# AlexanderGSC/gmres

Measured on AMD Instinct MI355X. Metric: Arnoldi iters/sec + HBM GB/s, 4096² Poisson-2D fp64, GMRES(m=95), higher is better.
Workload: dtype f64

## Files before the change

### gmres_amd/__init__.py

```python
from ._native import GkError, peer_info, runtime_info
from .solver import (MGSR_MF, MGSR_OMP, PREC, Context, LocalGroup, SolveResult, gmres_hh, gmres_mgsr, pbicgstab,
                     SrSolve, cb_plan_query, pcg, res_plan_query, slab_partition)

__all__ = ["GkError", "Context", "LocalGroup", "SolveResult", "gmres_mgsr", "gmres_hh", "slab_partition", "pcg", "pbicgstab", "MGSR_OMP", "MGSR_MF", "PREC",
           "res_plan_query", "cb_plan_query", "runtime_info", "SrSolve", "peer_info"]
```

### gmres_amd/_native.py

```python
from __future__ import annotations

import ctypes
import os
import sys
import re

PKG = os.path.dirname(os.path.abspath(__file__))
LIB_DIR = os.environ.get("GK_LIB_DIR") or os.path.join(PKG, "lib")
HIP_SO = os.path.join(LIB_DIR, "libgmres_hip.so")
FHOST_SO = os.path.join(LIB_DIR, "libgmres_fhost.so")
HEADER = os.path.join(os.path.dirname(PKG), "include", "gmres_hip.h")

GK_OK = 0
GK_ERR_COMM = -6
GK_TUNE_PROJ_NT = 0
GK_TUNE_STENCIL_BLOCKS = 2
GK_TUNE_SR_BLOCKS = 28
GK_TUNE_SR_TWO_LEVEL = 29
GK_TUNE_XCHG_TIMEOUT_MS = 7
GK_TUNE_RES, GK_TUNE_RES_R2, GK_TUNE_RES_SHARE, GK_TUNE_RES_TIMEOUT_MS = 8, 9, 10, 11
GK_TUNE_VERR_ORDER = 14
GK_TUNE_HH_FUSE = 15
GK_TUNE_CHEB_STEN = 16
GK_TUNE_SPIN_WAIT = 18
GK_TUNE_GRAPH = 19
GK_TUNE_RES_QDEF = 20
GK_TUNE_RES_PC = 21
GK_TUNE_RES_FOLD = 22
GK_TUNE_RES_BLOCK = 23
GK_TUNE_WATCHDOG_MS = 24
GK_TUNE_HH_NORM_ORDER = 25
GK_TUNE_RES_PF = 27
GK_TUNE_RES_PIPE = 30
GK_TUNE_RIGHT_FUSED = 31
GK_TUNE_RES_PIPE_CARRY = 32
GK_SIDE_LEFT, GK_SIDE_RIGHT = 0, 1
GK_BASIS_F64, GK_BASIS_F32 = 0, 1
GK_ERR_ARG, GK_ERR_STATE = -1, -4
GK_PREC_IDENTITY, GK_PREC_CBPR2, GK_PREC_CHEB = 0, 1, 2
(GK_KID_PROJ, GK_KID_STENCIL, GK_KID_SCALE, GK_KID_UPDATE, GK_KID_COMM, GK_KID_OTHER, GK_KID_RES, GK_KID_PREC,
 GK_KID_HALO, GK_KID_GRAPH) = range(10)
GK_KID_SR = 10
SR_PASS_NAMES = ["sr_cg_p", "sr_cg_x", "sr_cg_z", "sr_bi_p", "sr_bi_pc", "sr_bi_s", "sr_bi_sc", "sr_st1", "sr_st2",
                 "sr_bi_x", "sr_bi_pe", "sr_bi_se", "sr_dot", "sr_cg_xz", "sr_bi_pz", "sr_bi_sz"]
KID_NAMES = ["proj", "stencil", "scale", "update", "comm", "other", "res", "prec", "halo", "graph"] + SR_PASS_NAMES
GK_SR_PCG, GK_SR_BICGSTAB = 0, 1
COMM_KINDS = {0: None, 1: "rccl", 2: "local-group", 3: "xgmi-device-exchange"}
GK_RES_CB = 7
RES_VARIANTS = {0: None, 1: "prefetch", 2: "pairs", 3: "pairs+lds", 4: "w-only", 5: "w+column", 6: "blocked",
                GK_RES_CB: "compressed-basis"}
# ... 64 lines not shown
    "gk_hh_step_async": (c_int, [c_vp, c_int, c_int]),
    "gk_hh_step_wait": (c_int, [c_vp, c_int, _dp]),
    "gk_hh_update_x": (c_int, [c_vp, _dp, c_int]),
    "gk_hh_verr": (c_int, [c_vp, c_int, _dp]),
    "gk_profile_enable": (c_int, [c_vp, c_int]),
    "gk_profile_reset": (c_int, [c_vp]),
    "gk_profile_read": (c_int, [c_vp, c_int, _dp, ctypes.POINTER(c_ll)]),
    "gk_sync": (c_int, [c_vp]),
    "gk_debug_hold_stream": (c_int, [c_vp, c_int]),
    "gk_profile_res_wg": (c_int, [c_vp, c_int, _dp, _dp, c_int, _ip]),
    "gk_profile_res_trace": (c_int, [c_vp, c_int, c_int, c_int, c_vp, c_int, c_int, _ip, _ip, _dp]),
    "gk_profile_res_split": (c_int, [c_vp, c_int, c_int, _dp, _dp, _dp, ctypes.POINTER(c_ll)]),
    "gk_set_tuning": (c_int, [c_vp, c_int, c_int]),
    "gk_res_plan_query": (c_int, [c_ll, c_int, c_int, c_int, c_int, c_int, ctypes.POINTER(c_ll)]),
    "gk_res_info": (c_int, [c_vp, c_int, ctypes.POINTER(c_ll)]),
    "gk_lanczos_bounds": (c_int, [c_vp, c_int, _dp, _dp]),
    "gk_vec_count": (c_int, [c_vp, _ip]),
    "gk_vec_apply": (c_int, [c_vp, c_int, c_int, c_int]),
    "gk_vec_dot": (c_int, [c_vp, c_int, c_int, _dp]),
    "gk_vec_lincomb": (c_int, [c_vp, c_int, c_int, c_int, c_int, c_int, c_double, c_double]),
    "gk_sr_start": (c_int, [c_vp, c_int, c_double, c_int]),
    "gk_sr_iterate": (c_int, [c_vp, c_int]),
    "gk_sr_status": (c_int, [c_vp, c_int, _ip, _ip, _dp]),
    "gk_sr_history": (c_int, [c_vp, _dp, c_int]),
    "gk_poisson5": (c_int, [c_int, c_int, c_vp, c_vp, c_vp, c_vp, c_vp]),
    "gk_precond_apply": (c_int, [c_int, c_int, _dp, c_int, c_vp, c_vp, c_vp, c_vp]),
    "gk_mgs_project": (c_int, [c_ll, c_vp, c_vp, c_vp, c_vp]),
    "gk_dot": (c_int, [c_ll, c_vp, c_vp, c_vp, c_vp]),
}

# ... 123 lines not shown
```

### gmres_amd/csrc/gk_api.hip

```cpp
#include <dlfcn.h>

#include <algorithm>
#include <cmath>
#include <cstdarg>
#include <cstdio>
#include <cstdlib>
#include <cstring>

#include "gk_blk.hpp"
#include "gk_cb.hpp"
#include "gk_host.hpp"
#include "gk_kernels.hpp"
#include "gk_resident.hpp"

using namespace gkh;
using gk::nt_auto_for;
using gk::plan_info;
using gk::plan_resident;
using gk::ResPlan;
using gk::RES_R2_BIG;

namespace gkh __attribute__((visibility("hidden"))) {

thread_local std::string g_err;
// ... 233 lines not shown
bool res_plan(gk_ctx *c, ResPlan &p, bool hh = false) {
    if (c->tune_res == 0 || c->res_broken || c->m > gk::RHMAX || c->res_cus <= 0 || c->res_gath == nullptr)
        return false;
    if (collective(c) && !(c->xs_on && c->nranks > 1)) return false;
    if (c->tune_res < 0 && c->res_share > 1) return false;
    const int gmax = std::max(1, std::min(gk::RGMAX, c->res_cus / std::max(1, c->res_share)));
    const int cap = c->tune_res_r2 > 0 ? c->tune_res_r2 : RES_R2_BIG;
    plan_resident(c->nloc, gmax, cap, c->tune_res_wonly, hh,
                  c->tune_nt > 0 || (c->tune_nt < 0 && c->nt_auto), p, c->tune_res_pc, c->tune_res_blk, c->tune_res_pf,
                  c->tune_res_pipe, c->tune_res_carry);
    if (c->nranks > 1) p.carry = 0;
    if (p.wo && !hh && c->m + 1 > gk::WO_HMAX) return false;
    return true;
}

enum { RESF_CLOSE_HH = 1, RESF_UNIT_INIT = 2, RESF_PIN_LOCAL = 4 };
int res_step(gk_ctx *c, int j, const ResPlan &p, const double *pin, int npin, double *hs, double *hcopy,
             int mode = gk::RES_MGS, double *w = nullptr, i64 unit_g = -1, int flags = 0) {
    ProfScope ps(c, GK_KID_RES);
    const bool close = (flags & RESF_CLOSE_HH) && mode == gk::RES_HH_UP;
    if ((flags & ~RESF_PIN_LOCAL) != 0 && !p.wo)
        return set_err(GK_ERR_STATE, "resident flags %d need the w-only variant", flags);
    const bool pin_local = (flags & RESF_PIN_LOCAL) && mode != gk::RES_HH_DOWN && c->xs_on && c->nranks > 1;
    const int np = (mode == gk::RES_MGS ? (p.bvar >= 0 ? gk::blk_exchanges(j, p.blk) : 2 * j) : j) + (close ? 1 : 0);
    if (c->res_tag > 0xF0000000u) {
        HIPCHK(hipMemsetAsync(c->res_gath, 0, sizeof(gk::u64) * gk::RES_GATH_ALL, c->st));
        c->res_tag = 1;
    }
    gk::ResArgs a{};
    a.w = w != nullptr ? w : c->w;
    a.mode = mode;
    a.coef = mode == gk::RES_MGS ? 1.0 : 2.0;
    a.tail0 = mode == gk::RES_HH_UP ? (i64)j - c->g0 : 0;
    a.V = c->V;
    a.vout = c->V + (i64)j * c->ld;
    a.ld = c->ld;
    a.pin = pin;
    a.npin = npin;
    a.hs = hs;
    a.hcopy = hcopy;
    a.gath = c->res_gath;
    a.gm = c->res_gm;
    a.j = j;
    a.n = c->nloc;
    a.nres2 = p.nres2;
    a.r2e = p.r2e;
    a.l2e = p.l2e;
    a.unit_known = mode == gk::RES_HH_DOWN && unit_g >= 0;
    a.unit_e = (a.unit_known && unit_g >= c->g0 && unit_g < c->g0 + c->nloc) ? unit_g - c->g0 : -1;
    a.unit_init = a.unit_known && (flags & RESF_UNIT_INIT) ? 1 : 0;
    a.close_hh = close ? 1 : 0;
    a.hb = c->hb;
    a.tag0 = c->res_tag;
    c->res_tag += (unsigned)np;
    a.timeout = (gk::u64)c->res_timeout_ms * (gk::u64)c->xs_tick_per_ms;
    a.err = c->res_err_dev;
    a.stamps = c->res_split ? c->res_stamps : nullptr;
    if (c->res_trace != nullptr && j == c->res_trace_j && mode == c->res_trace_mode) {
        a.trace = c->res_trace;
        c->res_trace_g = p.G;
        c->res_trace_np = np;
    }
    a.qdef = c->tune_res_qdef != 0 ? 1 : 0;
    a.nranks = 1;
    if (c->xs_on && c->nranks > 1) {
        a.err = c->xs_err_dev;
        a.timeout = std::max(a.timeout, c->xs_timeout);
// ... 843 lines not shown
    CHK(check_ctx(c));
    if (j < 1 || j > c->m) return set_err(GK_ERR_ARG, "step j=%d outside 1..%d", j, c->m);
    if (!c->cycle_mgs) return set_err(GK_ERR_STATE, "gk_mgs_step before gk_mgs_cycle_start");
    HIPCHK(hipSetDevice(c->dev));
    const i64 ld = c->ld;
    double *V = c->V;
    const int m2 = c->m + 2;
    double *hs = c->hall + (i64)(j - 1) * m2;
    c->prof_on_step = (j % c->prof_every) == 0;
    const int s0 = 0;
    ResPlan rp;
    gk::CbPlan cp;
    const bool cb = cb_on(c);
    const bool res = cb ? cb_plan_ctx(c, cp) : res_plan(c, rp);
    const double *vj = cb ? cb_vjw(c) : V + (i64)(j - 1) * ld, *v1 = cb ? cb_v1w(c) : V;
    if (right_prec(c))
        CHK(op_right(c, vj, c->w, gk::ACC_DOT, v1, slot(c, s0)));
    else
        CHK(op_precond(c, vj, c->w, false, gk::ACC_DOT, v1, slot(c, s0)));
    int np = c->last_np;
    if (res && cb) {
        CHK(cb_step(c, j, cp, slot(c, s0), np, hs, c->hallh_dev + (i64)(j - 1) * m2));
        HIPCHK(hipEventRecord(c->ev_step[j], c->st));
        c->prof_on_step = true;
        return GK_OK;
    }
    if (res) {
        const bool fold = c->tune_res_fold && c->xs_on && c->nranks > 1;
        if (!fold) CHK(allreduce(c, slot(c, s0), np));
        CHK(res_step(c, j, rp, slot(c, s0), np, hs, c->hallh_dev + (i64)(j - 1) * m2, gk::RES_MGS, nullptr, -1,
// ... 376 lines not shown
            xs_set_timeout(c, value);
            break;
        case GK_TUNE_RES: c->tune_res = value < 0 ? -1 : (value != 0); break;
        case GK_TUNE_RES_R2:
            if (value != 0 && value != 2 && value != 4 && value != 8 && value != 12)
                return set_err(GK_ERR_ARG, "resident cap must be 0 (auto), 2, 4, 8 or 12");
            c->tune_res_r2 = value;
            break;
        case GK_TUNE_RES_SHARE:
            if (value < 1) return set_err(GK_ERR_ARG, "share must be >= 1");
            c->res_share = value;
            break;
        case GK_TUNE_RES_WONLY: c->tune_res_wonly = value < 0 ? -1 : (value != 0); break;
        case GK_TUNE_RES_PIPE: c->tune_res_pipe = value < 0 ? -1 : (value != 0); break;
        case GK_TUNE_RES_PIPE_CARRY: c->tune_res_carry = value < 0 ? -1 : (value != 0); break;
        case GK_TUNE_HH_FUSE: c->tune_hh_fuse = value != 0; break;
        case GK_TUNE_CHEB_STEN: c->tune_cheb_sten = value != 0; break;
        case GK_TUNE_SPIN_WAIT: c->tune_spin_wait = value != 0; break;
        case GK_TUNE_GRAPH: c->tune_graph = value != 0; break;
        case GK_TUNE_RES_QDEF: c->tune_res_qdef = value < 0 ? -1 : (value != 0); break;
        case GK_TUNE_RES_PC: c->tune_res_pc = value < 0 ? -1 : (value != 0); break;
        case GK_TUNE_RES_FOLD: c->tune_res_fold = value != 0; break;
        case GK_TUNE_WATCHDOG_MS: c->watchdog_ms = std::max(0, value); break;
        case GK_TUNE_HH_NORM_ORDER: c->tune_hh_norm_order = value != 0; break;
        case GK_TUNE_RES_BLOCK:
            if (value != 1 && value != 2 && value != 4)
                return set_err(GK_ERR_ARG, "GK_TUNE_RES_BLOCK %d: blocks of 1 (strict MGS-R), 2 or 4 projections", value);
            if (c->cycle_mgs)
                c->pend_res_blk = value;
            else
// ... 209 lines not shown
            info[gk::RPI_L2E] = cp.l2e;
            info[gk::RPI_LDS] = cp.lds;
            info[gk::RPI_NRES2] = cp.nres2;
            info[gk::RPI_WT] = gk::CB_WT;
            info[gk::RPI_BLK] = 1;
        }
    }
    int cs = c->pkind == GK_PREC_CHEB && c->tune_cheb_sten && c->pdeg <= gk::CF_LMAX && c->N >= gk::CF_PTS &&
             c->tune_cheb_fused && c->N % 2 == 0 &&
             (i64)c->N * std::max(c->nlines, c->max_lines) * 8 < (1LL << 31);
    if (cs && collective(c) && c->nranks > 1) cs = c->min_lines == 0 ? -1 : (c->min_lines >= c->pdeg + 1 ? 1 : 0);
    info[gk::RPI_CHEB_STEN] = cs;
    return GK_OK;
}

}


namespace gkh __attribute__((visibility("hidden"))) {
double *g_scratch[64] = {nullptr};

int stateless_ctx(gk_ctx &c, int N, int nlines, i64 n, void *stream) {
    int dev = 0;
    HIPCHK(hipGetDevice(&dev));
    if (dev < 0 || dev >= 64) return set_err(GK_ERR_ARG, "device id %d", dev);
    if (g_scratch[dev] == nullptr) {
        if (hipMalloc(&g_scratch[dev], sizeof(double) * (NSLOT * gk::NPMAX + 64)) != hipSuccess)
            return set_err(GK_ERR_NOMEM, "scratch allocation failed");
    }
    c.dev = dev;
// ... 248 lines not shown
```

### gmres_amd/csrc/gk_host.hpp

```cpp
#pragma once
#include <hip/hip_runtime.h>
#include <rccl/rccl.h>

#include <condition_variable>
#include <deque>
#include <mutex>
#include <string>
#include <vector>

#include "../../include/gmres_hip.h"
#include "gk_res.hpp"

using gk::i64;

namespace gk {
struct SrDev;
struct SrMirror;
}

struct gk_group {
    int n = 0;
    std::mutex mu;
    std::condition_variable cv;
    int arrived = 0;
// ... 51 lines not shown
    gk::u64 *res_gath = nullptr;
    double *res_gm = nullptr;
    int tune_res_blk = 1;
    int tune_res_pf = 0;
    int pend_res_blk = 0, pend_res_pf = -1;
    int watchdog_ms = 0;
    bool broken = false;
    unsigned *hold_word = nullptr, *hold_word_dev = nullptr;
    int *res_err = nullptr, *res_err_dev = nullptr;
    unsigned res_tag = 1;
    int res_cus = 0;
    int tune_res = -1;
    int tune_res_r2 = 0;
    int tune_res_pipe = -1;
    int tune_res_carry = -1;
    int tune_res_wonly = -1;
    int tune_verr_order = 1;
    int tune_hh_fuse = 1;
    int tune_hh_norm_order = 0;
    int res_share = 1;
    int res_timeout_ms = 20000;
    bool res_broken = false;
    gk::u64 *res_stamps = nullptr;
    bool res_split = false;
    gk::u64 *res_trace = nullptr;
    int res_trace_j = 0, res_trace_mode = -1;
    int res_trace_g = 0, res_trace_np = 0;
    int vec = 2, JT = 16;
    dim3 sgrid;
    int sr_JT = 64, tune_sr_blocks = 0;
// ... 117 lines not shown
```

### gmres_amd/csrc/gk_res.hpp

```cpp
#pragma once
#include "gk_common.hpp"
#include "gk_cheb.hpp"

namespace gk {

constexpr int XS_MAXR = 16;
constexpr int XS_MAXV = 128;
constexpr i64 XS_RED_WORDS = 2LL * XS_MAXR * XS_MAXV * 2;
typedef unsigned long long u64;
struct XsPeers {
    u64 *p[XS_MAXR];
};
enum { XS_SLAB = 0, XS_VEC = 1, XS_BCAST = 2 };

__device__ __forceinline__ void xs_put(u64 *q, unsigned seq, unsigned data) {
    __hip_atomic_store(q, ((u64)seq << 32) | data, __ATOMIC_RELAXED, __HIP_MEMORY_SCOPE_SYSTEM);
}

__device__ __forceinline__ int xs_flag(const int *err) {
    return __hip_atomic_load(err, __ATOMIC_RELAXED, __HIP_MEMORY_SCOPE_SYSTEM);
}

enum { XG_ABORT = -1, XG_LATE = 0, XG_OK = 1 };
__device__ __forceinline__ int xs_get(const u64 *q, unsigned seq, u64 deadline, unsigned *data, const int *err) {
// ... 39 lines not shown
    int unit_known;
    int r2e, l2e;
    XsPeers peers;
    int nranks, rank;
    unsigned xseq0;
    int mode;
    double coef;
    i64 tail0;
    u64 *stamps;
    int close_hh;
    double *hb;
    int unit_init;
    u64 *trace;
    int qdef;
    int pin_local;
    double *gm;
};
constexpr int RES_TRACE_X = 2 * RHMAX + 2;

struct ResClock {
    u64 t0 = 0, tp = 0, pass = 0, wait = 0;
    __device__ __forceinline__ void start(const u64 *st) {
        if (st != nullptr) t0 = tp = wall_clock64();
    }
    __device__ __forceinline__ void passed(const u64 *st) {
        if (st != nullptr) {
            const u64 n = wall_clock64();
            pass += n - tp;
            tp = n;
        }
    }
    __device__ __forceinline__ void waited(const u64 *st) {
        if (st != nullptr) {
            const u64 n = wall_clock64();
            wait += n - tp;
            tp = n;
        }
    }
    __device__ __forceinline__ void finish(u64 *st, int mode) {
        if (st != nullptr && threadIdx.x == 0) {
            u64 *q = st + 4 * ((i64)mode * RGMAX + blockIdx.x);
            q[0] += pass;
            q[1] += wait;
            q[2] += wall_clock64() - t0;
            q[3] += 1;
        }
    }
};

enum { RES_MGS = 0, RES_HH_UP = 1, RES_HH_DOWN = 2 };
enum { RK_NONE = 0, RK_DOT = 1, RK_NORM = 2 };

__device__ __forceinline__ unsigned res_stream_wg() { return gridDim.x - 1 - blockIdx.x; }
// ... 274 lines not shown
```

### gmres_amd/csrc/gk_resident.hip

```cpp
#include <hip/hip_runtime.h>

#include <algorithm>
#include <atomic>
#include <cstdarg>
#include <cstdio>

#include "../../include/gmres_hip.h"
#include "gk_blk.hpp"
#include "gk_res.hpp"
#include "gk_resident.hpp"

namespace gk {

template <int R2, int L2, bool PF, bool NT, bool CW, int MODE>
__global__ __launch_bounds__(RT, 2) void k_mgs_res(ResArgs a) {
    extern __shared__ double2 lw[];
    __shared__ double sm[RWAVES];
    __shared__ double bc[1];
    __shared__ int okf;
    __shared__ double hsh[RHMAX + 1];
    constexpr int RB = PF ? R2 : 1;
    constexpr int DT = CW ? RT - 64 : RT;
    const int t = threadIdx.x;
    const bool data = !CW || t >= 64;
// ... 291 lines not shown
static_assert(PIPE_CARRY >= 0 && PIPE_CARRY <= PIPE_D, "GK_RES_PIPE_CARRY: 0 .. GK_RES_PIPE_D chunks of the ring");
#ifndef GK_RES_TOUCH_MGS_CARRY
#define GK_RES_TOUCH_MGS_CARRY 20
#endif
constexpr int TOUCH_MGS_CARRY = GK_RES_TOUCH_MGS_CARRY;

template <class F, int... I>
__device__ __forceinline__ void seq_apply(F &&f, std::integer_sequence<int, I...>) {
    (f(std::integral_constant<int, I>{}), ...);
}
template <int N, class F>
__device__ __forceinline__ void seq_for(F &&f) {
    seq_apply(f, std::make_integer_sequence<int, N>{});
}

template <int RW, int LW, int MODE, int WBT = WB, bool PIPE = false, int CARRY = 0>
__global__ __launch_bounds__(WT, 1) void k_mgs_wres(ResArgs a) {
    static_assert(CARRY >= 0 && CARRY <= WBT && (CARRY == 0 || (PIPE && MODE == RES_MGS && CARRY <= RW)),
                  "carried chunks: a head of the pipelined pass's ring, register chunks of the MGS step");
    extern __shared__ double2 lw[];
    __shared__ double sm[WT / 64];
    __shared__ double bc[1];
    __shared__ int okf;
    __shared__ int xdone;
    __shared__ double hsh[MODE == RES_MGS ? WO_HMAX : 1];
    const int t = threadIdx.x;
    constexpr int mode = MODE;
    constexpr int PACE = MODE == RES_MGS ? TOUCH_PACE : TOUCH_PACE_HH;
    constexpr int TCH = MODE == RES_MGS ? (PIPE ? (CARRY > 0 ? TOUCH_MGS_CARRY : TOUCH_MGS_PIPE) : TOUCH_MGS) : TOUCH;
    const int j = a.j, np = res_np(mode, j);
    const i64 n2 = a.n >> 1, ld2 = a.ld >> 1;
    const i64 nch = a.nres2 / WT;
// ... 7 lines not shown
    clk.start(a.stamps);
    int touch_sink = 0;
    const i64 sstride = (i64)gridDim.x * WT;
    const i64 sbase = a.nres2 + (i64)res_stream_wg() * WT + t;
    double2 wr[RW];
    [[maybe_unused]] d2v ra[CARRY > 0 ? WBT : 1], rb[CARRY > 0 ? WBT : 1];
    if (mode == RES_HH_DOWN && a.unit_init) {
        const i64 u = a.unit_e;
        auto unit2 = [&](i64 e2) { return double2{2 * e2 == u ? 1.0 : 0.0, 2 * e2 + 1 == u ? 1.0 : 0.0}; };
#pragma unroll
        for (int k = 0; k < RW; ++k) wr[k] = (c0 + k < cend) ? unit2((c0 + k) * WT + t) : double2{0.0, 0.0};
        for (int k = 0; k < LW; ++k)
            if (l0 + k < lend) lw[k * WT + t] = unit2((l0 + k) * WT + t);
        for (i64 e = sbase; e < n2; e += sstride) W2[e] = unit2(e);
        if ((a.n & 1) && blockIdx.x == gridDim.x - 1 && t == 0) a.w[a.n - 1] = (a.n - 1 == u) ? 1.0 : 0.0;
    } else {
#pragma unroll
        for (int k = 0; k < RW; ++k) wr[k] = (PIPE || c0 + k < cend) ? W2[(c0 + k) * WT + t] : double2{0.0, 0.0};
        for (int k = 0; k < LW; ++k)
            if (PIPE || l0 + k < lend) lw[k * WT + t] = W2[(l0 + k) * WT + t];
    }
    auto red = [&](double &acc, const double2 &v, const double2 &b, int kind, i64 e2, bool chk) {
        if (kind == RK_DOT) {
            acc = acc + v.x * b.x;
            acc = acc + v.y * b.y;
        } else if (kind == RK_NORM) {
            sq_acc(acc, v, e2, tail0, chk);
        }
    };
    const i64 wc0 = c0, wl0 = l0;
// ... 130 lines not shown
                    wv[u].y = wv[u].y - ch * av[u].y;
                    W2[e] = wv[u];
                    red(acc, wv[u], bv[u], kind, e, mode == RES_HH_UP && 2 * a.nres2 < tail0);
                }
            }
        }
        if ((a.n & 1) && blockIdx.x == gridDim.x - 1 && t == 0) {
            const i64 e = a.n - 1;
            const double x = a.w[e] - ch * a.V[(i64)i * a.ld + e];
            a.w[e] = x;
            if (kind == RK_DOT) acc = acc + x * a.V[(i64)q * a.ld + e];
            if (kind == RK_NORM && e >= tail0) acc = acc + x * x;
        }
        return acc;
    };
    [[maybe_unused]] auto head = [&](int pn) {
        int zero = 0;
        asm volatile("" : "+s"(zero));
        const double2 *Ar = V2 + (i64)res_col(mode, j, pn) * ld2 + (wc0 + zero) * WT;
        const double2 *Br = V2 + (i64)res_col(mode, j, pn + 1) * ld2 + (wc0 + zero) * WT;
        const bool dot = pn < np - 1;
        const unsigned lo = (unsigned)t * (unsigned)sizeof(double2);
        seq_for<CARRY>([&](auto kc) {
            constexpr int k = decltype(kc)::value;
            const double2 *ap = Ar + k * WT;
            const double2 *bp = dot ? Br + k * WT : Ar;
            d2v &da = ra[k], &db = rb[k];
            const unsigned off = lo;
            asm volatile("global_load_dwordx4 %0, %1, %2 nt" : "=v"(da) : "v"(off), "s"(ap));
            asm volatile("global_load_dwordx4 %0, %1, %2" : "=v"(db) : "v"(off), "s"(bp));
// ... 50 lines not shown
        clk.waited(a.stamps);
        return okf != 0;
    };
    auto kind_of = [&](int p) { return p < np - 1 ? RK_DOT : (mode == RES_MGS ? RK_NORM : RK_NONE); };
    double h;
    bool ok = true;
    if (mode == RES_HH_DOWN) {
        const int q = res_col(mode, j, 0);
        double acc = 0.0;
        if (a.unit_known) {
            if (blockIdx.x == 0 && t == 0 && a.unit_e >= 0) acc = a.V[(i64)q * a.ld + a.unit_e];
        } else {
            acc = pass(0.0, q, q, RK_DOT);
        }
        ok = reduce(acc, h, kind_of(0) == RK_DOT ? res_col(mode, j, 1) : -1);
    } else {
        double s = 0.0;
        for (int k = t; k < a.npin; k += WT) s += a.pin[k];
        s = wave_sum(s);
        if ((t & 63) == 0) sm[t >> 6] = s;
        __syncthreads();
        h = sm[0];
#pragma unroll
        for (int w = 1; w < WT / 64; ++w) h += sm[w];
        __syncthreads();
        ok = res_pin_fold(a, h, bc, &okf);
    }
    if constexpr (CARRY > 0) {
        head(0);
        head_landed();
    }
    for (int p = 0; p < np && ok; ++p) {
        const int i = res_col(mode, j, p);
        const int kind = kind_of(p);
        if (mode == RES_MGS && blockIdx.x == 0 && t == 0) hsh[i] = (p < j ? 0.0 : hsh[i]) + h;
        const double acc = pass(mode == RES_MGS ? h : a.coef * h, i, res_col(mode, j, p + 1), kind);
        if (kind != RK_NONE)
            ok = reduce(acc, h, p + 1 < np && kind_of(p + 1) == RK_DOT ? res_col(mode, j, p + 2) : -1, p + 1);
    }
    if (!ok) return;
    const bool close = mode == RES_HH_UP && a.close_hh;
    if (mode != RES_MGS) {
        double acc = 0.0;
// ... 311 lines not shown
#define GK_RES_RW 89
#endif
#ifndef GK_RES_LW
#define GK_RES_LW 39
#endif
constexpr int RES_RW = GK_RES_RW, RES_LW = GK_RES_LW, RES_LW_HH = 38;
#ifndef GK_RES_RW_HH
#define GK_RES_RW_HH 90
#endif
constexpr int RES_RW_HH = GK_RES_RW_HH;
#ifndef GK_RES_PIPE
#define GK_RES_PIPE 1
#endif
constexpr bool RES_PIPE = GK_RES_PIPE != 0;
constexpr bool RES_PIPE_OK = 2 * (gk::PIPE_D - 1) <= 63 && RES_RW + RES_LW > gk::PIPE_D;

#ifndef GK_RES_PC_WB
#define GK_RES_PC_WB 4
#endif
#ifndef GK_RES_PC_WB_HH
#define GK_RES_PC_WB_HH 4
#endif
#ifndef GK_RES_PC_RX
#define GK_RES_PC_RX 4
#endif
constexpr int RES_PC_NT = 512;
#ifndef GK_RES_PC_RX_MGS
#define GK_RES_PC_RX_MGS 6
#endif
constexpr int RES_PC_RW = 32, RES_PC_RX = GK_RES_PC_RX, RES_PC_LX = 19;
// ... 161 lines not shown
    const int e = dyn_lds(reinterpret_cast<const void *>(&k_mgs_res<R2, L2, PF, NT, CW, MODE>), dev, p.lds, attr, msg);
    if (e != GK_OK) return e;
    k_mgs_res<R2, L2, PF, NT, CW, MODE><<<p.G, RT, p.lds, st>>>(a);
    return launched(msg);
}

template <int R2, int L2, bool PF, bool NT, bool CW>
int launch_res_t(const ResPlan &p, const ResArgs &a, int dev, hipStream_t st, std::string &msg) {
    switch (a.mode) {
        case RES_HH_UP: return launch_res_m<R2, L2, PF, NT, CW, RES_HH_UP>(p, a, dev, st, msg);
        case RES_HH_DOWN: return launch_res_m<R2, L2, PF, NT, CW, RES_HH_DOWN>(p, a, dev, st, msg);
        default: return launch_res_m<R2, L2, PF, NT, CW, RES_MGS>(p, a, dev, st, msg);
    }
}

template <int MODE, bool PIPE = false, int CARRY = 0>
int launch_wres_m(const ResPlan &p, const ResArgs &a, int dev, hipStream_t st, std::string &msg) {
    constexpr int RW = MODE == RES_MGS ? RES_RW : RES_RW_HH;
    constexpr int LW = MODE == RES_MGS ? RES_LW : RES_LW_HH;
    constexpr int WBT = PIPE ? PIPE_D : (MODE == RES_MGS ? WB : WB_HH);
    static std::atomic<int> attr[ATTR_DEVS];
    const int e =
        dyn_lds(reinterpret_cast<const void *>(&k_mgs_wres<RW, LW, MODE, WBT, PIPE, CARRY>), dev, p.lds, attr, msg);
    if (e != GK_OK) return e;
    k_mgs_wres<RW, LW, MODE, WBT, PIPE, CARRY><<<p.G, WT, p.lds, st>>>(a);
    return launched(msg);
}

int launch_wres(const ResPlan &p, const ResArgs &a, int dev, hipStream_t st, std::string &msg) {
    switch (a.mode) {
        case RES_HH_UP: return launch_wres_m<RES_HH_UP>(p, a, dev, st, msg);
        case RES_HH_DOWN: return launch_wres_m<RES_HH_DOWN>(p, a, dev, st, msg);
        default:
            if constexpr (RES_PIPE_OK) {
                if (p.pipe) {
                    if (p.r2e != RES_RW || p.l2e != RES_LW || (a.n & 1) || a.nres2 != a.n / 2)
                        return fail(msg, GK_ERR_STATE, "pipelined w-only step on a plan that is not full (%d + %d chunks)",
                                    p.r2e, p.l2e);
                    if constexpr (PIPE_CARRY > 0) {
                        if (p.carry != 0) {
                            if (a.nranks != 1 || p.carry != PIPE_CARRY)
                                return fail(msg, GK_ERR_STATE, "carried pass (%d chunks) on %d ranks", p.carry, a.nranks);
                            return launch_wres_m<RES_MGS, true, PIPE_CARRY>(p, a, dev, st, msg);
                        }
                    }
                    return launch_wres_m<RES_MGS, true>(p, a, dev, st, msg);
                }
            }
            return launch_wres_m<RES_MGS>(p, a, dev, st, msg);
    }
}

template <int RW, int RX, int LX, int MODE>
int launch_wpc_k(const ResPlan &p, const ResArgs &a, int dev, hipStream_t st, std::string &msg) {
    constexpr int WBT = MODE == RES_MGS ? RES_PC_WB : RES_PC_WB_HH;
    static std::atomic<int> attr[ATTR_DEVS];
    if (p.r2e > RW || p.lds < LX * RES_PC_NT * (int)sizeof(double2))
        return fail(msg, GK_ERR_STATE, "column-cache plan (%d chunks, %d B LDS) does not fit k_mgs_wpc<%d,%d,%d>", p.r2e,
                    p.lds, RW, RX, LX);
    const int e = dyn_lds(reinterpret_cast<const void *>(&k_mgs_wpc<RW, RX, LX, MODE, WBT, RES_PC_NT>), dev,
                          p.lds, attr, msg);
    if (e != GK_OK) return e;
    k_mgs_wpc<RW, RX, LX, MODE, WBT, RES_PC_NT><<<p.G, RES_PC_NT, p.lds, st>>>(a);
    return launched(msg);
// ... 44 lines not shown
```

### gmres_amd/csrc/gk_resident.hpp

```cpp
#pragma once
#include <string>

#include "gk_common.hpp"

namespace gk {

struct ResArgs;

constexpr int RES_R2_BIG = 12;

struct ResPlan {
    int G = 0, r2 = 0, l2 = 0;
    int r2e = 0, l2e = 0;
    bool pf = false, nt = false, cw = false, wo = false;
    bool pc = false;
    bool pcs = false;
    int blk = 0;
    int bvar = -1;
    int wt = 0;
    bool pipe = false;
    int carry = 0;
    i64 nres2 = 0;
    int lds = 0;
};

GK_HIDDEN i64 pc_bytes(i64 n2, int G, bool hh);
GK_HIDDEN i64 pairs_bytes(i64 n2, int G);
GK_HIDDEN i64 wonly_bytes(i64 n2, int G);

GK_HIDDEN void plan_resident(i64 nloc, int gmax, int cap, int tune_wonly, bool hh, bool nt, ResPlan &p,
                             int tune_pc = -1, int tune_blk = 1, int tune_pf = 0, int tune_pipe = -1,
                             int tune_carry = -1);
GK_HIDDEN bool nt_auto_for(i64 max_nloc);

enum { RPI_VARIANT = 0, RPI_G, RPI_R2, RPI_L2, RPI_PF, RPI_CW, RPI_WO, RPI_NT, RPI_R2E, RPI_L2E, RPI_LDS, RPI_NRES2, RPI_PIPE,
       RPI_CHEB_STEN, RPI_WT, RPI_BLK, RPI_CARRY };
GK_HIDDEN void plan_info(const ResPlan &p, bool on, long long *info);

GK_HIDDEN int res_launch(const ResPlan &p, const ResArgs &a, int dev, hipStream_t st, std::string &msg);

}
```

### gmres_amd/solver.py

```python
from __future__ import annotations

import ctypes
from dataclasses import dataclass, field

import numpy as np

from . import _native as nat

PREC = {"identity": nat.GK_PREC_IDENTITY, "none": nat.GK_PREC_IDENTITY,
        "cbpr2": nat.GK_PREC_CBPR2, "cheb": nat.GK_PREC_CHEB, "chebyshev": nat.GK_PREC_CHEB}
SIDE = {"left": nat.GK_SIDE_LEFT, "right": nat.GK_SIDE_RIGHT}
BASIS = {"f64": nat.GK_BASIS_F64, "f32": nat.GK_BASIS_F32}
MGSR_MF, MGSR_OMP = 0, 1


def _p(a: np.ndarray):
    assert a.dtype == np.float64 and a.flags["C_CONTIGUOUS"]
    return a.ctypes.data_as(nat._dp)


def slab_partition(N: int, nranks: int) -> list[tuple[int, int]]:
    if nranks < 1 or nranks > N:
        raise ValueError(f"cannot split {N} grid lines over {nranks} ranks")
    base, extra = divmod(N, nranks)
# ... 251 lines not shown
            nat.check(nat.hip().gk_profile_res_trace(self._h, int(arm), int(j), int(mode), None, 0, 0, None, None,
                                                     None), "gk_profile_res_trace")
            return None
        maxwg, maxx = 1024, 1026
        buf = np.zeros(maxwg * maxx * 2, dtype=np.uint64)
        g, x, tpm = ctypes.c_int(), ctypes.c_int(), ctypes.c_double()
        nat.check(nat.hip().gk_profile_res_trace(self._h, -1, 0, 0, buf.ctypes.data, maxwg, maxx, ctypes.byref(g),
                                                 ctypes.byref(x), ctypes.byref(tpm)), "gk_profile_res_trace")
        t = buf[: g.value * x.value * 2].reshape(g.value, x.value, 2).astype(np.float64)
        t0 = t[t > 0].min() if np.any(t > 0) else 0.0
        return (t[:, :, 0] - t0) / tpm.value, (t[:, :, 1] - t0) / tpm.value

    def res_info(self, hh: bool = False) -> dict:
        return _res_dict(lambda buf: nat.hip().gk_res_info(self._h, int(hh), buf), "gk_res_info")

    def tune(self, key: int, value: int) -> None:
        nat.check(nat.hip().gk_set_tuning(self._h, int(key), int(value)), "gk_set_tuning")

    def sync(self) -> None:
        nat.check(nat.hip().gk_sync(self._h), "gk_sync")

    def debug_hold_stream(self, hold: bool) -> None:
        nat.check(nat.hip().gk_debug_hold_stream(self._h, int(hold)), "gk_debug_hold_stream")


def _res_dict(call, what: str) -> dict:
    buf = (nat.c_ll * len(nat.RES_INFO_KEYS))()
    nat.check(call(buf), what)
    d = dict(zip(nat.RES_INFO_KEYS, (int(v) for v in buf)))
    d["variant"] = nat.RES_VARIANTS[d["variant"]]
    return d


def res_plan_query(nloc: int, cus: int = 256, share: int = 1, hh: bool = False, nt: int = -1,
                   block: int = 1) -> dict:
    return _res_dict(lambda buf: nat.hip().gk_res_plan_query(int(nloc), int(cus), int(share), int(hh), int(nt),
                                                             int(block), buf),
                     "gk_res_plan_query")


def cb_plan_query(nloc: int, cus: int = 256, share: int = 1, m: int = 95) -> dict:
    buf = (nat.c_ll * len(nat.CB_INFO_KEYS))()
    nat.check(nat.hip().gk_cb_plan_query(int(nloc), int(cus), int(share), int(m), buf), "gk_cb_plan_query")
    d = dict(zip(nat.CB_INFO_KEYS, (int(v) for v in buf)))
    d["on"] = bool(d["on"])
    return d


def _alloc_hist(m: int, max_cycles: int, want_hist: bool):
    if want_hist:
        return np.zeros(max_cycles), np.zeros(max_cycles * m)
    return np.zeros(1), np.zeros(1)

# ... 121 lines not shown
```

### include/gmres_hip.h

```cpp
#ifndef GMRES_HIP_H
#define GMRES_HIP_H

#ifdef __cplusplus
extern "C" {
#endif

#define GK_OK 0
#define GK_ERR_ARG (-1)
#define GK_ERR_HIP (-2)
#define GK_ERR_RCCL (-3)
#define GK_ERR_STATE (-4)
#define GK_ERR_NOMEM (-5)
#define GK_ERR_COMM (-6)

#define GK_PREC_IDENTITY 0
#define GK_PREC_CBPR2 1
#define GK_PREC_CHEB 2

#define GK_KID_PROJ 0
#define GK_KID_STENCIL 1
#define GK_KID_SCALE 2
#define GK_KID_UPDATE 3
#define GK_KID_COMM 4
#define GK_KID_OTHER 5
// ... 125 lines not shown
#define GK_TUNE_CHEB_STEN 16
#define GK_TUNE_SPIN_WAIT 18
#define GK_TUNE_GRAPH 19
#define GK_TUNE_RES_QDEF 20
#define GK_TUNE_RES_PC 21
#define GK_TUNE_RES_FOLD 22
#define GK_TUNE_RES_BLOCK 23
#define GK_TUNE_WATCHDOG_MS 24
#define GK_TUNE_HH_NORM_ORDER 25
#define GK_TUNE_RES_PF 27
#define GK_TUNE_SR_BLOCKS 28
#define GK_TUNE_SR_TWO_LEVEL 29
#define GK_TUNE_RES_PIPE 30
#define GK_TUNE_RIGHT_FUSED 31
#define GK_TUNE_RES_PIPE_CARRY 32
int gk_set_tuning(gk_ctx *ctx, int key, int value);
int gk_debug_hold_stream(gk_ctx *ctx, int hold);

int gk_poisson5(int nside, int nlines, const double *x, const double *halo_lo,
                const double *halo_hi, double *y, void *stream);
int gk_precond_apply(int nside, int kind, const double *params, int degree, const double *r,
                     double *z, double *scratch, void *stream);
int gk_mgs_project(long long n, double *w, const double *va, double *result, void *stream);
int gk_dot(long long n, const double *a, const double *b, double *result, void *stream);

#ifdef __cplusplus
}
#endif
#endif
```

Baseline: 272.2.

## Fuse Poisson stencil into the resident MGS kernel as a prologue

For single-rank, unpreconditioned, left-side Arnoldi on a square grid, the resident MGS-R kernel now applies the 5-point Poisson stencil to v_{j-1} itself. The stencil result is written directly into register and LDS chunks, and the first dot product with v_1 is computed in the same sweep. This removes the separate stencil launch and the HBM round trip of w. In exchange the kernel gains an extra exchange phase, a more complex sweep with shuffles and cross-line window loads, and extra register pressure. It is enabled by default when the plan fits, and a tuning key and probe API are added.

```diff
diff --git a/gmres_amd/__init__.py b/gmres_amd/__init__.py
--- a/gmres_amd/__init__.py
+++ b/gmres_amd/__init__.py
@@ -1,6 +1,6 @@
 from ._native import GkError, peer_info, runtime_info
 from .solver import (MGSR_MF, MGSR_OMP, PREC, Context, LocalGroup, SolveResult, gmres_hh, gmres_mgsr, pbicgstab,
-                     SrSolve, cb_plan_query, pcg, res_plan_query, slab_partition)
+                     SrSolve, cb_plan_query, pcg, res_plan_query, res_sten_query, slab_partition)
 
 __all__ = ["GkError", "Context", "LocalGroup", "SolveResult", "gmres_mgsr", "gmres_hh", "slab_partition", "pcg", "pbicgstab", "MGSR_OMP", "MGSR_MF", "PREC",
-           "res_plan_query", "cb_plan_query", "runtime_info", "SrSolve", "peer_info"]
+           "res_plan_query", "res_sten_query", "cb_plan_query", "runtime_info", "SrSolve", "peer_info"]
diff --git a/gmres_amd/_native.py b/gmres_amd/_native.py
--- a/gmres_amd/_native.py
+++ b/gmres_amd/_native.py
@@ -34,6 +34,7 @@
 GK_TUNE_RES_PIPE = 30
 GK_TUNE_RIGHT_FUSED = 31
 GK_TUNE_RES_PIPE_CARRY = 32
+GK_TUNE_RES_STEN = 33
 GK_SIDE_LEFT, GK_SIDE_RIGHT = 0, 1
 GK_BASIS_F64, GK_BASIS_F32 = 0, 1
 GK_ERR_ARG, GK_ERR_STATE = -1, -4
@@ -128,6 +129,9 @@
     "gk_set_tuning": (c_int, [c_vp, c_int, c_int]),
     "gk_res_plan_query": (c_int, [c_ll, c_int, c_int, c_int, c_int, c_int, ctypes.POINTER(c_ll)]),
     "gk_res_info": (c_int, [c_vp, c_int, ctypes.POINTER(c_ll)]),
+    "gk_res_sten_query": (c_int, [c_ll, c_int, c_int, c_int, c_int, c_int, c_int, c_int, c_int, c_int, c_int]),
+    "gk_res_sten_info": (c_int, [c_vp, c_int, _ip]),
+    "gk_res_sten_probe": (c_int, [c_vp, c_int]),
     "gk_lanczos_bounds": (c_int, [c_vp, c_int, _dp, _dp]),
     "gk_vec_count": (c_int, [c_vp, _ip]),
     "gk_vec_apply": (c_int, [c_vp, c_int, c_int, c_int]),
diff --git a/gmres_amd/csrc/gk_api.hip b/gmres_amd/csrc/gk_api.hip
--- a/gmres_amd/csrc/gk_api.hip
+++ b/gmres_amd/csrc/gk_api.hip
@@ -271,7 +271,13 @@
     return true;
 }
 
-enum { RESF_CLOSE_HH = 1, RESF_UNIT_INIT = 2, RESF_PIN_LOCAL = 4 };
+bool sten_ctx(const gk_ctx *c, const ResPlan &p) {
+    const bool plain = c->nranks == 1 && c->line0 == 0 && c->nlines == c->N && c->pkind == GK_PREC_IDENTITY &&
+                       c->side == GK_SIDE_LEFT && !cb_on(c) && c->tune_res_blk == 1;
+    return gk::plan_sten(p, c->nloc, c->N, false, plain, c->tune_res_sten);
+}
+
+enum { RESF_CLOSE_HH = 1, RESF_UNIT_INIT = 2, RESF_PIN_LOCAL = 4, RESF_STEN = 8, RESF_STEN_PROBE = 16 };
 int res_step(gk_ctx *c, int j, const ResPlan &p, const double *pin, int npin, double *hs, double *hcopy,
              int mode = gk::RES_MGS, double *w = nullptr, i64 unit_g = -1, int flags = 0) {
     ProfScope ps(c, GK_KID_RES);
@@ -279,7 +285,11 @@
     if ((flags & ~RESF_PIN_LOCAL) != 0 && !p.wo)
         return set_err(GK_ERR_STATE, "resident flags %d need the w-only variant", flags);
     const bool pin_local = (flags & RESF_PIN_LOCAL) && mode != gk::RES_HH_DOWN && c->xs_on && c->nranks > 1;
-    const int np = (mode == gk::RES_MGS ? (p.bvar >= 0 ? gk::blk_exchanges(j, p.blk) : 2 * j) : j) + (close ? 1 : 0);
+    const bool sten = (flags & RESF_STEN) != 0;
+    if (sten && (mode != gk::RES_MGS || !sten_ctx(c, p)))
+        return set_err(GK_ERR_STATE, "fused stencil prologue asked for outside its plan");
+    const int np = (mode == gk::RES_MGS ? (p.bvar >= 0 ? gk::blk_exchanges(j, p.blk) : 2 * j) : j) + (close ? 1 : 0) +
+                   (sten ? 1 : 0);
     if (c->res_tag > 0xF0000000u) {
         HIPCHK(hipMemsetAsync(c->res_gath, 0, sizeof(gk::u64) * gk::RES_GATH_ALL, c->st));
         c->res_tag = 1;
@@ -308,6 +318,8 @@
     a.unit_init = a.unit_known && (flags & RESF_UNIT_INIT) ? 1 : 0;
     a.close_hh = close ? 1 : 0;
     a.hb = c->hb;
+    a.sten_rc = sten ? c->N / 512 : 0;
+    a.sten_probe = sten && (flags & RESF_STEN_PROBE) ? 1 : 0;
     a.tag0 = c->res_tag;
     c->res_tag += (unsigned)np;
     a.timeout = (gk::u64)c->res_timeout_ms * (gk::u64)c->xs_tick_per_ms;
@@ -1181,6 +1193,12 @@
     const bool cb = cb_on(c);
     const bool res = cb ? cb_plan_ctx(c, cp) : res_plan(c, rp);
     const double *vj = cb ? cb_vjw(c) : V + (i64)(j - 1) * ld, *v1 = cb ? cb_v1w(c) : V;
+    if (res && !cb && sten_ctx(c, rp)) {
+        CHK(res_step(c, j, rp, nullptr, 0, hs, c->hallh_dev + (i64)(j - 1) * m2, gk::RES_MGS, nullptr, -1, RESF_STEN));
+        HIPCHK(hipEventRecord(c->ev_step[j], c->st));
+        c->prof_on_step = true;
+        return GK_OK;
+    }
     if (right_prec(c))
         CHK(op_right(c, vj, c->w, gk::ACC_DOT, v1, slot(c, s0)));
     else
@@ -1587,6 +1605,7 @@
         case GK_TUNE_RES_WONLY: c->tune_res_wonly = value < 0 ? -1 : (value != 0); break;
         case GK_TUNE_RES_PIPE: c->tune_res_pipe = value < 0 ? -1 : (value != 0); break;
         case GK_TUNE_RES_PIPE_CARRY: c->tune_res_carry = value < 0 ? -1 : (value != 0); break;
+        case GK_TUNE_RES_STEN: c->tune_res_sten = value == 0 ? 0 : -1; break;
         case GK_TUNE_HH_FUSE: c->tune_hh_fuse = value != 0; break;
         case GK_TUNE_CHEB_STEN: c->tune_cheb_sten = value != 0; break;
         case GK_TUNE_SPIN_WAIT: c->tune_spin_wait = value != 0; break;
@@ -1826,6 +1845,44 @@
     return GK_OK;
 }
 
+int gk_res_sten_query(long long nloc, int N, int cus, int share, int prec, int side, int nranks, int basis, int block,
+                      int hh, int key) {
+    if (nloc < 2 || N < 1 || cus < 1 || share < 1 || nranks < 1 || (block != 1 && block != 2 && block != 4)) {
+        set_err(GK_ERR_ARG, "bad fused-stencil query");
+        return 0;
+    }
+    const int gmax = std::max(1, std::min(gk::RGMAX, cus / share));
+    ResPlan p;
+    plan_resident(nloc, gmax, RES_R2_BIG, -1, hh != 0, nt_auto_for(nloc), p, -1, block);
+    const bool plain = nranks == 1 && nloc == (i64)N * N && prec == GK_PREC_IDENTITY && side == GK_SIDE_LEFT &&
+                       basis == GK_BASIS_F64 && block == 1;
+    return gk::plan_sten(p, nloc, N, hh != 0, plain, key) ? 1 : 0;
+}
+
+int gk_res_sten_info(gk_ctx *c, int hh, int *on) {
+    CHK(check_ctx(c));
+    if (on == nullptr) return set_err(GK_ERR_ARG, "null result");
+    ResPlan p;
+    *on = hh == 0 && !cb_on(c) && res_plan(c, p, false) && sten_ctx(c, p) ? 1 : 0;
+    return GK_OK;
+}
+
+int gk_res_sten_probe(gk_ctx *c, int j) {
+    CHK(check_ctx(c));
+    if (j < 1 || j > c->m) return set_err(GK_ERR_ARG, "step j=%d outside 1..%d", j, c->m);
+    if (!c->cycle_mgs) return set_err(GK_ERR_STATE, "gk_res_sten_probe before gk_mgs_cycle_start");
+    HIPCHK(hipSetDevice(c->dev));
+    ResPlan p;
+    if (cb_on(c) || !res_plan(c, p, false) || !sten_ctx(c, p))
+        return set_err(GK_ERR_STATE, "this context's MGS-R step does not run the fused stencil prologue");
+    const int m2 = c->m + 2;
+    CHK(res_step(c, j, p, nullptr, 0, c->hall + (i64)(j - 1) * m2, c->hallh_dev + (i64)(j - 1) * m2, gk::RES_MGS, nullptr,
+                 -1, RESF_STEN | RESF_STEN_PROBE));
+    HIPCHK(hipMemcpyAsync(c->V + (i64)j * c->ld, c->w, sizeof(double) * c->nloc, hipMemcpyDeviceToDevice, c->st));
+    HIPCHK(hipEventRecord(c->ev_step[j], c->st));
+    return GK_OK;
+}
+
 }
 
 
diff --git a/gmres_amd/csrc/gk_host.hpp b/gmres_amd/csrc/gk_host.hpp
--- a/gmres_amd/csrc/gk_host.hpp
+++ b/gmres_amd/csrc/gk_host.hpp
@@ -89,6 +89,7 @@
     int tune_res_r2 = 0;
     int tune_res_pipe = -1;
     int tune_res_carry = -1;
+    int tune_res_sten = -1;
     int tune_res_wonly = -1;
     int tune_verr_order = 1;
     int tune_hh_fuse = 1;
diff --git a/gmres_amd/csrc/gk_res.hpp b/gmres_amd/csrc/gk_res.hpp
--- a/gmres_amd/csrc/gk_res.hpp
+++ b/gmres_amd/csrc/gk_res.hpp
@@ -77,6 +77,8 @@
     u64 *trace;
     int qdef;
     int pin_local;
+    int sten_rc;
+    int sten_probe;
     double *gm;
 };
 constexpr int RES_TRACE_X = 2 * RHMAX + 2;
@@ -100,6 +102,7 @@
             tp = n;
         }
     }
+    __device__ __forceinline__ void not_a_projection() { pass = wait = 0; }
     __device__ __forceinline__ void finish(u64 *st, int mode) {
         if (st != nullptr && threadIdx.x == 0) {
             u64 *q = st + 4 * ((i64)mode * RGMAX + blockIdx.x);
diff --git a/gmres_amd/csrc/gk_resident.hip b/gmres_amd/csrc/gk_resident.hip
--- a/gmres_amd/csrc/gk_resident.hip
+++ b/gmres_amd/csrc/gk_resident.hip
@@ -329,8 +329,9 @@
     seq_apply(f, std::make_integer_sequence<int, N>{});
 }
 
-template <int RW, int LW, int MODE, int WBT = WB, bool PIPE = false, int CARRY = 0>
+template <int RW, int LW, int MODE, int WBT = WB, bool PIPE = false, int CARRY = 0, bool STEN = false>
 __global__ __launch_bounds__(WT, 1) void k_mgs_wres(ResArgs a) {
+    static_assert(!STEN || MODE == RES_MGS, "the fused stencil prologue is the MGS step's");
     static_assert(CARRY >= 0 && CARRY <= WBT && (CARRY == 0 || (PIPE && MODE == RES_MGS && CARRY <= RW)),
                   "carried chunks: a head of the pipelined pass's ring, register chunks of the MGS step");
     extern __shared__ double2 lw[];
@@ -368,6 +369,11 @@
             if (l0 + k < lend) lw[k * WT + t] = unit2((l0 + k) * WT + t);
         for (i64 e = sbase; e < n2; e += sstride) W2[e] = unit2(e);
         if ((a.n & 1) && blockIdx.x == gridDim.x - 1 && t == 0) a.w[a.n - 1] = (a.n - 1 == u) ? 1.0 : 0.0;
+    } else if constexpr (STEN) {
+        const double2 *__restrict__ J2 = V2 + (i64)(j - 1) * ld2;
+#pragma unroll
+        for (int k = 0; k < RW; ++k) wr[k] = J2[(c0 + k) * WT + t];
+        for (int k = 0; k < LW; ++k) lw[k * WT + t] = J2[(l0 + k) * WT + t];
     } else {
 #pragma unroll
         for (int k = 0; k < RW; ++k) wr[k] = (PIPE || c0 + k < cend) ? W2[(c0 + k) * WT + t] : double2{0.0, 0.0};
@@ -528,6 +534,102 @@
         }
         return acc;
     };
+    [[maybe_unused]] auto sten_sweep = [&]() -> double {
+        constexpr int SB = PIPE ? 8 : 4;
+        constexpr int WN = 8;
+        const int rc = a.sten_rc;
+        const double2 *__restrict__ J2 = V2 + (i64)(j - 1) * ld2;
+        const double *__restrict__ Jd = a.V + (i64)(j - 1) * a.ld;
+        const int lane = t & 63;
+        const int eoff = lane < 32 ? 2 * (t - lane) - 1 : 2 * (t - lane) + 128;
+        auto pick = [&](const double2 x1, const double2 x2, const double2 x4, const double2 x8) {
+            const bool r8 = rc == 8, r4 = rc == 4, r2 = rc == 2;
+            return double2{r8 ? x8.x : (r4 ? x4.x : (r2 ? x2.x : x1.x)), r8 ? x8.y : (r4 ? x4.y : (r2 ? x2.y : x1.y))};
+        };
+        double acc = 0.0;
+        auto range = [&](auto regc, const i64 b0, const i64 bend) {
+            constexpr bool REG = decltype(regc)::value;
+            constexpr int NC = REG ? RW : LW;
+            static_assert(NC >= WN, "a range at least as long as the window");
+            double2 win[WN];
+            {
+                int zero = 0;
+                asm volatile("" : "+s"(zero));
+                const i64 b = b0 + zero;
+#pragma unroll
+                for (int r = 0; r < WN; ++r) {
+                    const i64 c = b - WN + r;
+                    const double2 v = J2[(c < 0 ? 0 : c) * WT + t];
+                    win[r] = c < 0 ? double2{0.0, 0.0} : v;
+                }
+            }
+            auto batch = [&](const int k0, auto nbc) {
+                constexpr int NB = decltype(nbc)::value;
+                __builtin_amdgcn_sched_barrier(0);
+                int zero = 0;
+                asm volatile("" : "+s"(zero));
+                const i64 b = b0 + zero;
+                double2 b1[NB], hn[NB];
+                double ed[NB];
+#pragma unroll
+                for (int u = 0; u < NB; ++u) {
+                    const int k = k0 + u;
+                    if (k < NC) {
+                        b1[u] = V2[(b + k) * WT + t];
+                        if (k + WN >= NC) {
+                            const i64 c = b + k + rc;
+                            const double2 v = J2[(c < nch ? c : nch - 1) * WT + t];
+                            hn[u] = c < nch ? v : double2{0.0, 0.0};
+                        }
+                        const int eo = (b + k == 0 && eoff < 0) ? 0 : eoff;
+                        ed[u] = (Jd + (b + k) * (2 * WT))[eo];
+                    }
+                }
+                __builtin_amdgcn_sched_barrier(0);
+#pragma unroll
+                for (int u = 0; u < NB; ++u) {
+                    const int k = k0 + u;
+                    if (k < NC && b + k < bend) {
+                        double2 c, nx;
+                        if constexpr (REG) {
+                            c = wr[k];
+                            nx = pick(wr[k + 1 < NC ? k + 1 : k], wr[k + 2 < NC ? k + 2 : k], wr[k + 4 < NC ? k + 4 : k],
+                                      wr[k + 8 < NC ? k + 8 : k]);
+                        } else {
+                            c = lw[k * WT + t];
+                            nx = lw[(k + rc < NC ? k + rc : k) * WT + t];
+                        }
+                        if (k + WN >= NC) {
+                            if (k + rc >= NC) nx = hn[u];
+                        }
+                        const double2 pv = pick(win[(k + WN - 1) % WN], win[(k + WN - 2) % WN], win[(k + WN - 4) % WN],
+                                                win[k % WN]);
+                        double left = __shfl_up(c.y, 1, 64), right = __shfl_down(c.x, 1, 64);
+                        if (lane == 0) left = ed[u];
+                        if (lane == 63) right = ed[u];
+                        const int col = ((int)(b0 + k) & (rc - 1)) * (2 * WT) + 2 * t;
+                        if (col == 0) left = 0.0;
+                        if (col + 2 == rc * 2 * WT) right = 0.0;
+                        const double sx = ((left + c.y) + nx.x) + pv.x;
+                        const double sy = ((c.x + right) + nx.y) + pv.y;
+                        const double2 wv{4.0 * c.x - 1.0 * sx, 4.0 * c.y - 1.0 * sy};
+                        win[k % WN] = c;
+                        if constexpr (REG) wr[k] = wv; else lw[k * WT + t] = wv;
+                        acc = acc + wv.x * b1[u].x;
+                        acc = acc + wv.y * b1[u].y;
+                    }
+                }
+            };
+            constexpr int NCM = (NC - WN) / SB * SB;
+#pragma unroll
+            for (int k0 = 0; k0 < NCM; k0 += SB) batch(k0, std::integral_constant<int, SB>{});
+#pragma unroll
+            for (int k0 = NCM; k0 < NC; k0 += SB / 2) batch(k0, std::integral_constant<int, SB / 2>{});
+        };
+        range(std::true_type{}, c0, cend);
+        range(std::false_type{}, l0, lend);
+        return acc;
+    };
     [[maybe_unused]] auto head = [&](int pn) {
         int zero = 0;
         asm volatile("" : "+s"(zero));
@@ -608,6 +710,21 @@
             acc = pass(0.0, q, q, RK_DOT);
         }
         ok = reduce(acc, h, kind_of(0) == RK_DOT ? res_col(mode, j, 1) : -1);
+    } else if constexpr (STEN) {
+        const double acc = sten_sweep();
+        ok = reduce(acc, h, res_col(mode, j, 1), 0);
+        clk.not_a_projection();
+        if (a.sten_probe) {
+            if (!ok) return;
+#pragma unroll
+            for (int k = 0; k < RW; ++k) W2[(c0 + k) * WT + t] = wr[k];
+            for (int k = 0; k < LW; ++k) W2[(l0 + k) * WT + t] = lw[k * WT + t];
+            if (blockIdx.x == 0 && t == 0) {
+                a.hs[0] = h;
+                a.hcopy[0] = h;
+            }
+            return;
+        }
     } else {
         double s = 0.0;
         for (int k = t; k < a.npin; k += WT) s += a.pin[k];
@@ -620,7 +737,7 @@
         __syncthreads();
         ok = res_pin_fold(a, h, bc, &okf);
     }
-    if constexpr (CARRY > 0) {
+    if constexpr (CARRY > 0 && !STEN) {
         head(0);
         head_landed();
     }
@@ -962,6 +1079,21 @@
 #endif
 constexpr bool RES_PIPE = GK_RES_PIPE != 0;
 constexpr bool RES_PIPE_OK = 2 * (gk::PIPE_D - 1) <= 63 && RES_RW + RES_LW > gk::PIPE_D;
+#ifndef GK_RES_STEN
+#define GK_RES_STEN 1
+#endif
+constexpr bool RES_STEN = GK_RES_STEN != 0;
+constexpr bool RES_STEN_OK = RES_RW >= 8 && RES_LW >= 8;
+
+bool plan_sten(const ResPlan &p, i64 nloc, int N, bool hh, bool plain, int tune_sten) {
+    if (!RES_STEN_OK || hh || !plain || !(tune_sten < 0 ? RES_STEN : tune_sten != 0)) return false;
+    const i64 n2 = nloc / 2;
+    const bool full = p.wo && p.bvar < 0 && !p.pc && p.r2e == RES_RW && p.l2e == RES_LW && nloc % 2 == 0 &&
+                      n2 == (i64)p.G * (RES_RW + RES_LW) * gk::WT && p.nres2 == n2;
+    if (!full || N < 512 || N % 512 != 0 || nloc % N != 0) return false;
+    const int rc = N / 512;
+    return rc == 1 || rc == 2 || rc == 4 || rc == 8;
+}
 
 #ifndef GK_RES_PC_WB
 #define GK_RES_PC_WB 4
@@ -1153,17 +1285,25 @@
     }
 }
 
-template <int MODE, bool PIPE = false, int CARRY = 0>
+template <int MODE, bool PIPE = false, int CARRY = 0, bool STEN = false>
 int launch_wres_m(const ResPlan &p, const ResArgs &a, int dev, hipStream_t st, std::string &msg) {
     constexpr int RW = MODE == RES_MGS ? RES_RW : RES_RW_HH;
     constexpr int LW = MODE == RES_MGS ? RES_LW : RES_LW_HH;
     constexpr int WBT = PIPE ? PIPE_D : (MODE == RES_MGS ? WB : WB_HH);
     static std::atomic<int> attr[ATTR_DEVS];
-    const int e =
-        dyn_lds(reinterpret_cast<const void *>(&k_mgs_wres<RW, LW, MODE, WBT, PIPE, CARRY>), dev, p.lds, attr, msg);
+    const int e = dyn_lds(reinterpret_cast<const void *>(&k_mgs_wres<RW, LW, MODE, WBT, PIPE, CARRY, STEN>), dev, p.lds,
+                          attr, msg);
     if (e != GK_OK) return e;
-    k_mgs_wres<RW, LW, MODE, WBT, PIPE, CARRY><<<p.G, WT, p.lds, st>>>(a);
+    k_mgs_wres<RW, LW, MODE, WBT, PIPE, CARRY, STEN><<<p.G, WT, p.lds, st>>>(a);
     return launched(msg);
+}
+
+template <bool PIPE = false, int CARRY = 0>
+int launch_wres_s(const ResPlan &p, const ResArgs &a, int dev, hipStream_t st, std::string &msg) {
+    if constexpr (RES_STEN_OK) {
+        if (a.sten_rc > 0) return launch_wres_m<RES_MGS, PIPE, CARRY, true>(p, a, dev, st, msg);
+    }
+    return launch_wres_m<RES_MGS, PIPE, CARRY>(p, a, dev, st, msg);
 }
 
 int launch_wres(const ResPlan &p, const ResArgs &a, int dev, hipStream_t st, std::string &msg) {
@@ -1171,6 +1311,15 @@
         case RES_HH_UP: return launch_wres_m<RES_HH_UP>(p, a, dev, st, msg);
         case RES_HH_DOWN: return launch_wres_m<RES_HH_DOWN>(p, a, dev, st, msg);
         default:
+            if (a.sten_rc != 0) {
+                const i64 nch = a.nres2 / WT;
+                const int rc = a.sten_rc;
+                if (!RES_STEN_OK || (rc != 1 && rc != 2 && rc != 4 && rc != 8) || p.r2e != RES_RW || p.l2e != RES_LW ||
+                    (a.n & 1) || a.nres2 != a.n / 2 || nch != (i64)p.G * (RES_RW + RES_LW) || nch % rc != 0 ||
+                    a.nranks != 1)
+                    return fail(msg, GK_ERR_STATE, "fused stencil prologue on a plan it does not fit (%d chunks per line)",
+                                rc);
+            }
             if constexpr (RES_PIPE_OK) {
                 if (p.pipe) {
                     if (p.r2e != RES_RW || p.l2e != RES_LW || (a.n & 1) || a.nres2 != a.n / 2)
@@ -1180,13 +1329,13 @@
                         if (p.carry != 0) {
                             if (a.nranks != 1 || p.carry != PIPE_CARRY)
                                 return fail(msg, GK_ERR_STATE, "carried pass (%d chunks) on %d ranks", p.carry, a.nranks);
-                            return launch_wres_m<RES_MGS, true, PIPE_CARRY>(p, a, dev, st, msg);
+                            return launch_wres_s<true, PIPE_CARRY>(p, a, dev, st, msg);
                         }
                     }
-                    return launch_wres_m<RES_MGS, true>(p, a, dev, st, msg);
-                }
-            }
-            return launch_wres_m<RES_MGS>(p, a, dev, st, msg);
+                    return launch_wres_s<true>(p, a, dev, st, msg);
+                }
+            }
+            return launch_wres_s<>(p, a, dev, st, msg);
     }
 }
 
diff --git a/gmres_amd/csrc/gk_resident.hpp b/gmres_amd/csrc/gk_resident.hpp
--- a/gmres_amd/csrc/gk_resident.hpp
+++ b/gmres_amd/csrc/gk_resident.hpp
@@ -32,6 +32,7 @@
                              int tune_pc = -1, int tune_blk = 1, int tune_pf = 0, int tune_pipe = -1,
                              int tune_carry = -1);
 GK_HIDDEN bool nt_auto_for(i64 max_nloc);
+GK_HIDDEN bool plan_sten(const ResPlan &p, i64 nloc, int N, bool hh, bool plain, int tune_sten);
 
 enum { RPI_VARIANT = 0, RPI_G, RPI_R2, RPI_L2, RPI_PF, RPI_CW, RPI_WO, RPI_NT, RPI_R2E, RPI_L2E, RPI_LDS, RPI_NRES2, RPI_PIPE,
        RPI_CHEB_STEN, RPI_WT, RPI_BLK, RPI_CARRY };
diff --git a/gmres_amd/solver.py b/gmres_amd/solver.py
--- a/gmres_amd/solver.py
+++ b/gmres_amd/solver.py
@@ -289,6 +289,19 @@
     def res_info(self, hh: bool = False) -> dict:
         return _res_dict(lambda buf: nat.hip().gk_res_info(self._h, int(hh), buf), "gk_res_info")
 
+    def res_sten(self, hh: bool = False) -> int:
+        v = ctypes.c_int()
+        nat.check(nat.hip().gk_res_sten_info(self._h, int(hh), ctypes.byref(v)), "gk_res_sten_info")
+        return v.value
+
+    def res_sten_probe(self, j: int) -> None:
+        nat.check(nat.hip().gk_res_sten_probe(self._h, int(j)), "gk_res_sten_probe")
+
+    def mgs_step_wait(self, j: int) -> np.ndarray:
+        h = np.zeros(j + 1)
+        nat.check(nat.hip().gk_mgs_step_wait(self._h, j, _p(h)), "gk_mgs_step_wait")
+        return h
+
     def tune(self, key: int, value: int) -> None:
         nat.check(nat.hip().gk_set_tuning(self._h, int(key), int(value)), "gk_set_tuning")
 
@@ -312,6 +325,14 @@
     return _res_dict(lambda buf: nat.hip().gk_res_plan_query(int(nloc), int(cus), int(share), int(hh), int(nt),
                                                              int(block), buf),
                      "gk_res_plan_query")
+
+
+def res_sten_query(N: int, cus: int = 256, share: int = 1, prec: str | int = "identity", side: str = "left",
+                   nranks: int = 1, basis: str = "f64", block: int = 1, hh: bool = False, key: int = -1,
+                   nloc: int | None = None) -> int:
+    k = PREC[prec] if isinstance(prec, str) else int(prec)
+    return int(nat.hip().gk_res_sten_query(int(N * N if nloc is None else nloc), int(N), int(cus), int(share), k,
+                                           SIDE[side], int(nranks), BASIS[basis], int(block), int(hh), int(key)))
 
 
 def cb_plan_query(nloc: int, cus: int = 256, share: int = 1, m: int = 95) -> dict:
diff --git a/include/gmres_hip.h b/include/gmres_hip.h
--- a/include/gmres_hip.h
+++ b/include/gmres_hip.h
@@ -163,7 +163,12 @@
 #define GK_TUNE_RES_PIPE 30
 #define GK_TUNE_RIGHT_FUSED 31
 #define GK_TUNE_RES_PIPE_CARRY 32
+#define GK_TUNE_RES_STEN 33
 int gk_set_tuning(gk_ctx *ctx, int key, int value);
+int gk_res_sten_query(long long nloc, int N, int cus, int share, int prec, int side, int nranks, int basis, int block,
+                      int hh, int key);
+int gk_res_sten_info(gk_ctx *ctx, int hh, int *on);
+int gk_res_sten_probe(gk_ctx *ctx, int j);
 int gk_debug_hold_stream(gk_ctx *ctx, int hold);
 
 int gk_poisson5(int nside, int nlines, const double *x, const double *halo_lo,
```

New measurement: 274.8 (median of 6 runs). Within noise of the previous version (+0.9%).
